# microsoft/hivedscheduler

Hardware: AMD Instinct MI355X
Metric: scheduling p50 latency + VC-safety violations; RCCL bus-bw at 1/2/4/8-GPU cells (lower is better)
Workload: dtype fp32; 1 GPU; model=hived-sched-config4-fragmentation-stress, cluster=simulated 4-node x 8-MI355X, global_batch=64, seq_len=0, parallelism=single

## Files before the change

hivedscheduler_amd/core/algorithm.cpp:

```cpp
#include <cstdio>
#include <cstdlib>

#include "core.hpp"

namespace hived {

bool mapDebugRelease() {
  static int v = -1;
  if (v < 0) v = getenv("HIVED_DEBUG_MAP") ? 1 : 0;
  return v == 1;
}

namespace {
constexpr size_t kWaitReasonReserve = 128;

using OverlappingPreemptors = std::vector<Group*>;

OverlappingPreemptors collectPreemptionVictims(const Placement<PhysicalCell>& placement,
                                               VictimList* victims) {
  OverlappingPreemptors overlapping;
  victims->clear();
  for (auto& [leafNum, pods] : placement) {
    (void)leafNum;
    for (auto& pod : pods) {
// ... 79 lines not shown

int getAllocatedPodIndex(const BindInfo& info, int leafCellNum) {
  for (auto& mbi : info.memberBindInfo) {
    if (mbi.empty() || static_cast<int>(mbi[0].leafIndices.size()) != leafCellNum) continue;
    for (size_t podIndex = 0; podIndex < mbi.size(); podIndex++) {
      auto& pl = mbi[podIndex];
      if (pl.node == info.node && !info.isolation.empty() &&
          std::find(pl.leafIndices.begin(), pl.leafIndices.end(), info.isolation[0]) !=
              pl.leafIndices.end()) {
        return static_cast<int>(podIndex);
      }
    }
  }
  return -1;
}

bool allPodsReleased(const FlatLeafMap<PodSlots>& allocatedPods) {
  for (auto& [ln, pods] : allocatedPods) {
    (void)ln;
    for (auto& p : pods) {
      if (p.present) return false;
    }
  }
  return true;
}

bool anyBoundUnder(PhysicalCell* c) {
  if (c->virt != nullptr) return true;
  for (Cell* ch : c->children) {
    if (anyBoundUnder(static_cast<PhysicalCell*>(ch))) return true;
  }
  return false;
}

void initGroup(Group* g, const PodSpec& s, GState state) {
  g->name = s.groupName;
  g->vc = s.vc;
  g->lazyPreemptionEnable = s.lazyPreemptionEnable;
  g->ignoreK8sSuggestedNodes = s.ignoreK8sSuggestedNodes;
  g->gangReleaseEnable = s.gangReleaseEnable;
  g->priority = s.priority;
  g->state = state;
  g->totalPodNums = s.groupPodNums;
  for (auto& [leafNum, podNum] : s.groupPodNums) {
    g->allocatedPods[leafNum].resize(podNum);
    g->physPlacement[leafNum].assign(podNum, leafNum);
    g->virtPlacement[leafNum].assign(podNum, leafNum);
  }
}

}


ScheduleResult HivedCore::schedule(const PodSpec& s, const std::string& podKey,
                                   const std::set<std::string>& suggestedNodes, Phase phase) {
  OpGuard opGuard(this);
  scheduleCount_++;
  Placement<PhysicalCell> phys;
  Placement<VirtualCell> virt;
  bool hasVirtual = true;
  VictimList& victims = victimScratch_;
  victims.clear();
  std::string waitReason;
  waitReason.reserve(kWaitReasonReserve);
  int podIndex = 0;
  bool havePlacement = false;

  Group* g = nullptr;
  if (auto it = groups_.find(s.groupName); it != groups_.end()) g = it->second.get();
  if (g != nullptr) {
    havePlacement = schedulePodFromExistingGroup(g, s, suggestedNodes, phase, podKey, &phys,
                                                 &hasVirtual, &virt, &victims, &podIndex);
    if (!havePlacement) {
      auto it = groups_.find(s.groupName);
      g = it == groups_.end() ? nullptr : it->second.get();
    }
  }
  if (g == nullptr) {
    g = schedulePodFromNewGroup(s, suggestedNodes, phase, podKey, &phys, &hasVirtual, &virt,
                                &victims, &waitReason);
    havePlacement = !phys.empty();
  }
  (void)havePlacement;
  return generateResult(phys, hasVirtual, virt, victims, std::move(waitReason), s.leafCellNumber,
                        podIndex, g, s.groupName);
}

ScheduleResult HivedCore::generateResult(const Placement<PhysicalCell>& phys, bool hasVirtual,
                                         const Placement<VirtualCell>& virt,
                                         const VictimList& victims,
                                         std::string&& waitReason, int currentLeafNum,
                                         int podIndex, Group* group,
                                         const std::string& groupName) {
  ScheduleResult r;
  if (phys.empty()) {
    r.kind = ScheduleResult::Kind::Wait;
    if (waitReason.empty()) {
      r.waitReason = "waiting for resources";
    } else {
      r.waitReason = std::move(waitReason);
    }
    return r;
  }
  if (!victims.empty()) {
    r.kind = ScheduleResult::Kind::Preempt;
    victims.nodeAt(victimRng_() % victims.nodeCount(), &r.victimNode, &r.victimPodKeys);
    return r;
  }
  r.kind = ScheduleResult::Kind::Bind;
  auto built = std::make_shared<BindInfo>();
  BindInfo& info = *built;
  info.memberBindInfo.reserve(phys.size());
  for (auto& [leafNum, pods] : phys) {
    std::vector<PodPlacementInfo> placements(pods.size());
    for (size_t pi = 0; pi < pods.size(); pi++) {
      auto& pl = placements[pi];
      pl.leafIndices.assign(leafNum, 0);
      pl.preassignedTypes.assign(leafNum, "");
      for (int li = 0; li < leafNum; li++) {
        PhysicalCell* c = pods[pi][li];
        if (c == nullptr) {
          if (group == nullptr || group->state == GState::Preempting) {
// ... 336 lines not shown
      .append(" node");
  return false;
}

bool HivedCore::chainHasBadLinks(const ChainCellList& ccl) {
  for (Cell* c : ccl.at(ccl.top())) {
    if (static_cast<PhysicalCell*>(c)->badLinksUnder > 0) return true;
  }
  return false;
}

std::map<std::string, Placement<VirtualCell>> HivedCore::tryLazyPreempt(
    const Placement<VirtualCell>& p, const std::string& groupName) {
  std::map<std::string, Placement<VirtualCell>> preempted;
  for (auto& [leafNum, pods] : p) {
    (void)leafNum;
    for (auto& pod : pods) {
      for (VirtualCell* leaf : pod) {
        if (PhysicalCell* pc = leaf->phys) {
          if (pc->state == CState::Used && pc->usingGroup->lazyPreemptionEnable &&
              !preempted.count(pc->usingGroup->name)) {
            preempted[pc->usingGroup->name] = lazyPreemptGroup(pc->usingGroup, groupName);
          }
        }
      }
    }
  }
  return preempted;
}

bool HivedCore::scheduleOpportunisticGroup(const SchedulingRequest& sr,
                                           Placement<PhysicalCell>* phys,
                                           std::string* failedReason) {
  if (!sr.topo->Schedule(sr.podLeafCellNums, kOpportunisticPriority, *sr.suggestedNodes,
                         sr.ignoreSuggestedNodes, phys, failedReason, sr.hbmBytes)) {
    failedReason->append(" when scheduling in physical cluster");
    return false;
  }
  return true;
}


void HivedCore::deleteUnallocatedPod(const PodSpec& s, const std::string& podKey) {
  OpGuard opGuard(this);
  auto it = groups_.find(s.groupName);
  if (it == groups_.end() || it->second->state != GState::Preempting) return;
  Group* g = it->second.get();
  g->preemptingPods.erase(podKey);
  if (g->preemptingPods.empty()) {
    deletePreemptingGroup(g, podKey);
  }
}

void HivedCore::addAllocatedPod(const PodSpec& s, const BindInfo& info, const std::string& podKey) {
  addAllocatedPodShared(s, info, nullptr, podKey);
}

void HivedCore::addAllocatedPod(const PodSpec& s, const std::shared_ptr<const BindInfo>& info,
                                const std::string& podKey) {
  addAllocatedPodShared(s, *info, &info, podKey);
}

void HivedCore::addAllocatedPodShared(const PodSpec& s, const BindInfo& info,
                                      const std::shared_ptr<const BindInfo>* shared,
                                      const std::string& podKey) {
  OpGuard opGuard(this);
  int podIndex = 0;
  bool releasable = true;
  Group* g = nullptr;
  auto it = groups_.find(s.groupName);
  if (it != groups_.end()) {
    g = it->second.get();
    if (g->state == GState::Preempting) allocatePreemptingGroup(g, podKey);
    podIndex = getAllocatedPodIndex(info, s.leafCellNumber);
    if (podIndex == -1) return;
  } else {
    g = createAllocatedGroup(s, info, podKey);
    podIndex = getAllocatedPodIndex(info, s.leafCellNumber);
    if (podIndex == -1) {
      podIndex = 0;
      releasable = false;
    }
  }
  setPodSlot(g, s.leafCellNumber, podIndex, releasable, podKey,
             shared != nullptr ? *shared : std::make_shared<const BindInfo>(info));
}

void HivedCore::deleteAllocatedPod(const PodSpec& s, const BindInfo& info,
                                   const std::string& podKey) {
  OpGuard opGuard(this);
  auto it = groups_.find(s.groupName);
  if (it == groups_.end()) return;
  Group* g = it->second.get();
  int podIndex = getAllocatedPodIndex(info, s.leafCellNumber);
  if (podIndex == -1) return;
  clearPodSlot(g, s.leafCellNumber, podIndex);
  if (allPodsReleased(g->allocatedPods)) {
    deleteAllocatedGroup(g, podKey);
  }
}

bool HivedCore::deleteAllocatedPodByKey(const std::string& podKey) {
  auto it = podIndex_.find(podKey);
  if (it == podIndex_.end()) return false;
  const PodSlotRef ref = it->second;
  OpGuard opGuard(this);
  if (!ref.releasable) return true;
  podIndex_.erase(it);
  ref.group->allocatedPods[ref.leafCellNum][ref.podIndex] = AllocatedPod{};
  if (allPodsReleased(ref.group->allocatedPods)) {
    deleteAllocatedGroup(ref.group, podKey);
  }
  return true;
}

void HivedCore::setPodSlot(Group* g, int leafCellNum, int podIndex, bool releasable,
                           const std::string& podKey, std::shared_ptr<const BindInfo> info) {
  auto& slots = g->allocatedPods[leafCellNum];
  if (podIndex >= static_cast<int>(slots.size())) slots.resize(podIndex + 1);
  AllocatedPod& slot = slots[podIndex];
  if (slot.present && slot.key != podKey) clearPodSlot(g, leafCellNum, podIndex);
  slot.present = true;
  slot.key = podKey;
  slot.node = info->node;
  slot.bindInfo = std::move(info);
  podIndex_[podKey] = PodSlotRef{g, leafCellNum, podIndex, releasable};
}

void HivedCore::clearPodSlot(Group* g, int leafCellNum, int podIndex) {
  auto& slots = g->allocatedPods[leafCellNum];
  if (podIndex >= static_cast<int>(slots.size())) return;
  AllocatedPod& slot = slots[podIndex];
  if (slot.present) {
    auto it = podIndex_.find(slot.key);
    if (it != podIndex_.end() && it->second.group == g &&
        it->second.leafCellNum == leafCellNum && it->second.podIndex == podIndex) {
      podIndex_.erase(it);
    }
// ... 442 lines not shown
```

hivedscheduler_amd/core/bindings.cpp:

```cpp
#include <pybind11/pybind11.h>
#include <pybind11/stl.h>

#include <climits>
#include <cstring>
#include <functional>
#include <mutex>

#include "core.hpp"

namespace py = pybind11;
using namespace hived;

namespace {

std::string dstr(const py::dict& d, const char* key, const std::string& def = "") {
  if (!d.contains(key)) return def;
  py::object v = d[key];
  if (v.is_none()) return def;
  return py::cast<std::string>(py::str(v));
}
long long dint(const py::dict& d, const char* key, long long def = 0) {
  if (!d.contains(key)) return def;
  py::object v = d[key];
  if (v.is_none()) return def;
// ... 115 lines not shown
};
Names N{};

PyObject* internName(const char* s) {
  PyObject* o = PyUnicode_InternFromString(s);
  if (o == nullptr) throw py::error_already_set();
  return o;
}

void initNames() {
#define HIVED_NAME(x) N.x = internName(#x)
  HIVED_NAME(virtualCluster);
  HIVED_NAME(priority);
  HIVED_NAME(pinnedCellId);
  HIVED_NAME(leafCellType);
  HIVED_NAME(leafCellNumber);
  HIVED_NAME(gangReleaseEnable);
  HIVED_NAME(lazyPreemptionEnable);
  HIVED_NAME(ignoreK8sSuggestedNodes);
  HIVED_NAME(hbmBytesPerCell);
  HIVED_NAME(affinityGroup);
  HIVED_NAME(name);
  HIVED_NAME(members);
  HIVED_NAME(podNumber);
  HIVED_NAME(node);
  HIVED_NAME(cellChain);
  HIVED_NAME(leafCellIsolation);
  HIVED_NAME(affinityGroupBindInfo);
  HIVED_NAME(podPlacements);
  HIVED_NAME(physicalNode);
  HIVED_NAME(physicalLeafCellIndices);
  HIVED_NAME(preassignedCellTypes);
  HIVED_NAME(kind);
  HIVED_NAME(bind);
  HIVED_NAME(preempt);
  HIVED_NAME(wait);
  HIVED_NAME(bindInfo);
  HIVED_NAME(victimNode);
  HIVED_NAME(victimPodKeys);
  HIVED_NAME(reason);
  HIVED_NAME(pod_spec);
  HIVED_NAME(spec);
  HIVED_NAME(pod_key);
  HIVED_NAME(suggested_nodes);
  HIVED_NAME(phase);
  HIVED_NAME(commit);
  HIVED_NAME(validate);
  HIVED_NAME(Filtering);
  HIVED_NAME(Preempting);
  HIVED_NAME(code);
#undef HIVED_NAME
}

struct ApiTypes {
  PyObject* PodSchedulingSpec;
  PyObject* AffinityGroupSpec;
  PyObject* AffinityGroupMemberSpec;
  PyObject* PodBindInfo;
  PyObject* AffinityGroupMemberBindInfo;
  PyObject* PodPlacementInfo;
  PyObject* WebServerError;
  PyObject* emptyTuple;
  PyObject* one;
};
ApiTypes T{};

void initApiTypes() {
  py::module_ types = py::module_::import("hivedscheduler_amd.api.types");
#define HIVED_TYPE(x) T.x = py::object(types.attr(#x)).release().ptr()
  HIVED_TYPE(PodSchedulingSpec);
  HIVED_TYPE(AffinityGroupSpec);
  HIVED_TYPE(AffinityGroupMemberSpec);
  HIVED_TYPE(PodBindInfo);
  HIVED_TYPE(AffinityGroupMemberBindInfo);
  HIVED_TYPE(PodPlacementInfo);
  HIVED_TYPE(WebServerError);
#undef HIVED_TYPE
  T.emptyTuple = PyTuple_New(0);
  T.one = PyLong_FromLong(1);
  if (T.emptyTuple == nullptr || T.one == nullptr) throw py::error_already_set();
}

class Record {
 public:
  explicit Record(py::handle rec) : rec_(rec.ptr()) {
    if (PyDict_Check(rec_)) {
      dict_ = rec_;
      wire_ = true;
      return;
    }
    PyObject* tp = reinterpret_cast<PyObject*>(Py_TYPE(rec_));
    if (tp == T.PodSchedulingSpec || tp == T.AffinityGroupMemberSpec ||
        tp == T.AffinityGroupSpec) {
      dict_ = ownedDict_ = PyObject_GenericGetDict(rec_, nullptr);
      if (dict_ == nullptr) PyErr_Clear();
    }
  }
  Record(const Record&) = delete;
  Record& operator=(const Record&) = delete;
  ~Record() { Py_XDECREF(ownedDict_); }
  py::handle object() const { return rec_; }

 private:
  friend class Field;
  PyObject* rec_;
  PyObject* dict_ = nullptr;
// ... 252 lines not shown
};

py::dict bindInfoToDict(const BindInfo& info, const NameStrs& names) {
  py::dict d;
  setItem(d, N.node, names.str(info.node));
  setItem(d, N.leafCellIsolation, pyIntList(info.isolation));
  setItem(d, N.cellChain, names.str(info.chain));
  py::list mbis(info.memberBindInfo.size());
  for (size_t m = 0; m < info.memberBindInfo.size(); m++) {
    auto& mbi = info.memberBindInfo[m];
    py::list placements(mbi.size());
    for (size_t p = 0; p < mbi.size(); p++) {
      auto& pl = mbi[p];
      py::dict pd;
      setItem(pd, N.physicalNode, names.str(pl.node));
      setItem(pd, N.physicalLeafCellIndices, pyIntList(pl.leafIndices));
      setItem(pd, N.preassignedCellTypes, names.strList(pl.preassignedTypes));
      PyList_SET_ITEM(placements.ptr(), static_cast<Py_ssize_t>(p), pd.release().ptr());
    }
    py::dict md;
    setItem(md, N.podPlacements, placements);
    PyList_SET_ITEM(mbis.ptr(), static_cast<Py_ssize_t>(m), md.release().ptr());
  }
  setItem(d, N.affinityGroupBindInfo, mbis);
  return d;
}

bool isNodeNameCollection(py::handle v) {
  PyObject* o = v.ptr();
  if (PySequence_Check(o) != 0) return !PyUnicode_Check(o) && !PyBytes_Check(o);
  if (PyGen_Check(o) != 0 || PyAnySet_Check(o) != 0) return true;
  if (PyType_Check(o)) return false;
  const char* tp = Py_TYPE(o)->tp_name;
  for (const char* ok : {"dict_keys", "dict_values", "dict_items", "map", "zip"}) {
    if (std::strcmp(tp, ok) == 0) return true;
  }
  return false;
}

std::set<std::string> toNodeNameSet(py::handle v) {
  std::set<std::string> out;
  Items items(v);
  for (Py_ssize_t i = 0; i < items.size(); i++) {
    py::handle item = items[i];
    if (!PyUnicode_Check(item.ptr()) && !PyBytes_Check(item.ptr())) {
      throw py::type_error("suggested_nodes must contain node names (str)");
    }
    out.insert(py::cast<std::string>(item));
  }
  return out;
}


py::object newInstance(PyObject* cls) {
  PyTypeObject* tp = reinterpret_cast<PyTypeObject*>(cls);
  PyObject* o = tp->tp_new(tp, T.emptyTuple, nullptr);
  if (o == nullptr) throw py::error_already_set();
  return py::reinterpret_steal<py::object>(o);
}
void setAttr(py::handle o, PyObject* name, py::handle value) {
  if (PyObject_SetAttr(o.ptr(), name, value.ptr()) != 0) throw py::error_already_set();
}

py::object defaultAffinityGroup(py::handle podKey, py::handle leafCellNumber) {
  py::object member = newInstance(T.AffinityGroupMemberSpec);
  setAttr(member, N.podNumber, T.one);
  setAttr(member, N.leafCellNumber, leafCellNumber);
  py::list members(1);
  PyList_SET_ITEM(members.ptr(), 0, member.release().ptr());
  py::object group = newInstance(T.AffinityGroupSpec);
  setAttr(group, N.name, podKey);
  setAttr(group, N.members, members);
  return group;
}

PodSpec parseValidatedPodSpec(py::handle spec, py::handle podKey, const std::string& key) {
  if (PyDict_Check(spec.ptr())) {
    throw py::type_error("schedule_pod validates a PodSchedulingSpec object, not a dict");
  }
  Record d(spec);
  PodSpec s;
  Field leaf(d, N.leafCellNumber);
  bool defaulted = false;
  {
    Field ag(d, N.affinityGroup);
    if (!ag) {
      setAttr(spec, N.affinityGroup, defaultAffinityGroup(podKey, leaf.get()));
      defaulted = true;
    }
  }
  s.vc = fstr(d, N.virtualCluster);
  if (s.vc.empty()) throw HivedError::BadRequest("VirtualCluster is empty");
  long long priority = fint(d, N.priority);
  if (priority < kOpportunisticPriority) {
    throw HivedError::BadRequest("Priority is less than " + std::to_string(kOpportunisticPriority));
  }
  if (priority > kMaxGuaranteedPriority) {
    throw HivedError::BadRequest("Priority is greater than " +
                                 std::to_string(kMaxGuaranteedPriority));
  }
  s.priority = static_cast<int>(priority);
  long long leafNum = leaf ? toLongLong(leaf.get()) : 0;
  if (leafNum <= 0) throw HivedError::BadRequest("LeafCellNumber is non-positive");
  s.leafCellNumber = static_cast<int>(leafNum);
  if (defaulted) {
    s.groupName = key;
    s.groupPodNums[s.leafCellNumber] = 1;
  } else {
    Field ag(d, N.affinityGroup);
    Record group(ag.get());
    s.groupName = fstr(group, N.name);
    if (s.groupName.empty()) throw HivedError::BadRequest("AffinityGroup.Name is empty");
    bool podInGroup = false;
    if (Field members{group, N.members}) {
      Items ms(members.get());
      for (Py_ssize_t i = 0; i < ms.size(); i++) {
        Record member(ms[i]);
        long long podNumber = fint(member, N.podNumber);
        if (podNumber <= 0) {
          throw HivedError::BadRequest("AffinityGroup.Members has non-positive PodNumber");
        }
        long long memberLeafNum = fint(member, N.leafCellNumber);
        if (memberLeafNum <= 0) {
          throw HivedError::BadRequest("AffinityGroup.Members has non-positive LeafCellNumber");
        }
        if (memberLeafNum == leafNum) podInGroup = true;
        s.groupPodNums[static_cast<int>(memberLeafNum)] += static_cast<int>(podNumber);
      }
    }
    if (!podInGroup) {
      throw HivedError::BadRequest("AffinityGroup.Members does not contain current Pod");
    }
  }
  s.pinnedCellId = fstr(d, N.pinnedCellId);
  s.leafCellType = fstr(d, N.leafCellType);
  s.gangReleaseEnable = fbool(d, N.gangReleaseEnable, false);
  s.lazyPreemptionEnable = fbool(d, N.lazyPreemptionEnable, false);
  s.ignoreK8sSuggestedNodes = fbool(d, N.ignoreK8sSuggestedNodes, true);
  s.hbmBytesPerCell = fint(d, N.hbmBytesPerCell);
  if (s.hbmBytesPerCell < 0) {
    throw HivedError::BadRequest("hbmBytesPerCell must be non-negative");
  }
  return s;
}

py::object bindInfoToObject(const BindInfo& info, const NameStrs& names) {
  py::list mbis(info.memberBindInfo.size());
  for (size_t m = 0; m < info.memberBindInfo.size(); m++) {
    auto& mbi = info.memberBindInfo[m];
    py::list placements(mbi.size());
    for (size_t p = 0; p < mbi.size(); p++) {
      auto& pl = mbi[p];
      py::object po = newInstance(T.PodPlacementInfo);
      setAttr(po, N.physicalNode, names.str(pl.node));
      setAttr(po, N.physicalLeafCellIndices, pyIntList(pl.leafIndices));
      setAttr(po, N.preassignedCellTypes, names.strList(pl.preassignedTypes));
      PyList_SET_ITEM(placements.ptr(), static_cast<Py_ssize_t>(p), po.release().ptr());
    }
    py::object mo = newInstance(T.AffinityGroupMemberBindInfo);
    setAttr(mo, N.podPlacements, placements);
    PyList_SET_ITEM(mbis.ptr(), static_cast<Py_ssize_t>(m), mo.release().ptr());
  }
  py::object o = newInstance(T.PodBindInfo);
  setAttr(o, N.node, names.str(info.node));
  setAttr(o, N.leafCellIsolation, pyIntList(info.isolation));
  setAttr(o, N.cellChain, names.str(info.chain));
  setAttr(o, N.affinityGroupBindInfo, mbis);
  return o;
}

struct PyScheduleResult {
  PyObject_HEAD
  PyObject* bindInfo;
  PyObject* victimNode;
  PyObject* victimPodKeys;
  PyObject* waitReason;
  hived::ScheduleResult r;
  std::shared_ptr<const NameStrs> names;
};

void resultDealloc(PyObject* self) {
  auto* o = reinterpret_cast<PyScheduleResult*>(self);
  Py_XDECREF(o->bindInfo);
  Py_XDECREF(o->victimNode);
  Py_XDECREF(o->victimPodKeys);
  Py_XDECREF(o->waitReason);
  o->r.~ScheduleResult();
  o->names.~shared_ptr();
  Py_TYPE(self)->tp_free(self);
}

template <class Make>
PyObject* cachedAttr(PyObject** slot, Make make) {
  if (*slot == nullptr) {
    try {
      *slot = make().release().ptr();
    } catch (py::error_already_set& e) {
      e.restore();
      return nullptr;
    } catch (const std::exception& e) {
      PyErr_SetString(PyExc_RuntimeError, e.what());
      return nullptr;
    }
  }
  Py_INCREF(*slot);
  return *slot;
}

PyObject* resultKind(PyObject* self, void*) {
  PyObject* k = nullptr;
  switch (reinterpret_cast<PyScheduleResult*>(self)->r.kind) {
    case hived::ScheduleResult::Kind::Bind: k = N.bind; break;
    case hived::ScheduleResult::Kind::Preempt: k = N.preempt; break;
    case hived::ScheduleResult::Kind::Wait: k = N.wait; break;
  }
  Py_INCREF(k);
  return k;
}
PyObject* resultBindInfo(PyObject* self, void*) {
  auto* o = reinterpret_cast<PyScheduleResult*>(self);
  if (o->r.kind != hived::ScheduleResult::Kind::Bind) Py_RETURN_NONE;
// ... 253 lines not shown
    if (!isNodeNameCollection(suggestedNodes)) {
      throw py::type_error("suggested_nodes must be a sequence of node names, not " +
                           std::string(Py_TYPE(suggestedNodes.ptr())->tp_name));
    }
    PodSpec s = parsePodSpec(spec);
    bool needSuggested = !s.ignoreK8sSuggestedNodes;
    if (!needSuggested) {
      CoreSection section(coreMutex_);
      auto it = core_.groups().find(s.groupName);
      needSuggested = it != core_.groups().end() && !it->second->ignoreK8sSuggestedNodes;
    }
    std::set<std::string> suggested;
    if (needSuggested) suggested = toNodeNameSet(suggestedNodes);
    Phase ph = (phase == "Preempting") ? Phase::Preempting : Phase::Filtering;
    ScheduleResult r = [&] {
      CoreSection section(coreMutex_);
      return core_.schedule(s, podKey, suggested, ph);
    }();
    py::dict d;
    switch (r.kind) {
      case ScheduleResult::Kind::Bind:
        setItem(d, N.kind, N.bind);
        setItem(d, N.bindInfo, bindInfoToDict(*r.bindInfo, *nameStrs_));
        break;
      case ScheduleResult::Kind::Preempt:
        setItem(d, N.kind, N.preempt);
        setItem(d, N.victimNode, pyStr(r.victimNode));
        setItem(d, N.victimPodKeys, pyStrList(r.victimPodKeys));
        break;
      case ScheduleResult::Kind::Wait:
        setItem(d, N.kind, N.wait);
        setItem(d, N.reason, pyStr(r.waitReason));
        break;
    }
    return d;
  }

  py::object schedulePod(py::handle spec, py::handle podKey, py::handle suggestedNodes,
                         py::handle phase, bool commit, bool validate) {
    if (!PyUnicode_Check(podKey.ptr())) throw py::type_error("pod_key must be a str");
    Phase ph = Phase::Filtering;
    if (phase.ptr() != nullptr && phase.ptr() != N.Filtering) {
      if (!PyUnicode_Check(phase.ptr())) throw py::type_error("phase must be a str");
      if (phase.ptr() == N.Preempting ||
          PyUnicode_CompareWithASCIIString(phase.ptr(), "Preempting") == 0) {
        ph = Phase::Preempting;
      }
    }
    if (!suggestedNodes.is_none() && !isNodeNameCollection(suggestedNodes)) {
      throw py::type_error("suggested_nodes must be a sequence of node names, not " +
                           std::string(Py_TYPE(suggestedNodes.ptr())->tp_name));
    }
    std::string key = toStdString(podKey);
    PodSpec s = validate ? parseValidatedPodSpec(spec, podKey, key) : parsePodSpec(spec);
    bool needSuggested = !s.ignoreK8sSuggestedNodes;
    if (!needSuggested) {
      CoreSection section(coreMutex_);
      auto it = core_.groups().find(s.groupName);
      needSuggested = it != core_.groups().end() && !it->second->ignoreK8sSuggestedNodes;
    }
    std::set<std::string> given;
    const std::set<std::string>* suggested = &given;
    if (needSuggested) {
      if (suggestedNodes.is_none()) {
        suggested = &allNodeSet_;
      } else {
        given = toNodeNameSet(suggestedNodes);
      }
    }
    hived::ScheduleResult r = [&] {
      CoreSection section(coreMutex_);
      hived::ScheduleResult decided = core_.schedule(s, key, *suggested, ph);
      if (commit && decided.kind == hived::ScheduleResult::Kind::Bind) {
        core_.addAllocatedPod(s, decided.bindInfo, key);
      }
      return decided;
    }();
    return makeResult(std::move(r), nameStrs_);
  }

  void deleteUnallocatedPod(py::handle spec, const std::string& podKey) {
    PodSpec s = parsePodSpec(spec);
    CoreSection section(coreMutex_);
    core_.deleteUnallocatedPod(s, podKey);
  }
  void addAllocatedPod(py::handle spec, py::handle bindInfo, const std::string& podKey) {
    PodSpec s = parsePodSpec(spec);
    BindInfo info = parseBindInfo(bindInfo);
    CoreSection section(coreMutex_);
    core_.addAllocatedPod(s, info, podKey);
  }
  void deleteAllocatedPod(py::handle spec, py::handle bindInfo, const std::string& podKey) {
    PodSpec s = parsePodSpec(spec);
    BindInfo info = parseBindInfo(bindInfo);
    CoreSection section(coreMutex_);
    core_.deleteAllocatedPod(s, info, podKey);
  }

  bool deleteAllocatedPodByKey(py::handle podKey) {
    if (!PyUnicode_Check(podKey.ptr())) throw py::type_error("pod_key must be a str");
    Py_ssize_t n = 0;
    const char* utf8 = PyUnicode_AsUTF8AndSize(podKey.ptr(), &n);
    if (utf8 == nullptr) throw py::error_already_set();
    CoreSection section(coreMutex_);
    releaseKey_.assign(utf8, static_cast<size_t>(n));
    return core_.deleteAllocatedPodByKey(releaseKey_);
  }

  py::list getAllAffinityGroups() const {
    py::list out;
    for (auto& [name, g] : core_.groups()) {
      (void)name;
      out.append(groupToDict(g.get()));
    }
    return out;
  }

  py::dict getAffinityGroup(const std::string& name) const {
    auto it = core_.groups().find(name);
    if (it == core_.groups().end()) {
      throw HivedError::BadRequest("Affinity group " + name +
                                   " does not exist since it is not allocated or preempting");
    }
    return groupToDict(it->second.get());
  }

  py::dict getClusterStatus() {
    py::dict d;
    d["physicalCluster"] = getPhysicalClusterStatus();
    d["virtualClusters"] = getAllVirtualClustersStatus();
    return d;
// ... 45 lines not shown
      (void)chain;
      for (Cell* c : st.full.at(kLowestLevel)) {
        auto* pc = static_cast<PhysicalCell*>(c);
        if (pc->otVC == vcName) {
          py::dict d;
          d["cellType"] = pc->typeName;
          d["cellAddress"] = pc->address + "-opp";
          d["cellState"] = to_string(CState::Used);
          d["cellHealthiness"] = pc->healthy ? "Healthy" : "Bad";
          d["cellPriority"] = kOpportunisticPriority;
          d["physicalCell"] = pc->address;
          out.append(d);
        }
      }
    }
    return out;
  }

  long long scheduleCount() const { return core_.scheduleCount_; }
  void checkInvariants() const { hived::checkInvariants(core_); }

  py::dict debugCounters() const {
    py::dict d;
    for (auto& [chain, st] : core_.chainStates_) {
      py::dict cd;
      for (int level = kLowestLevel; level <= st.top; level++) {
        py::dict ld;
        ld["totalLeft"] = st.totalLeft[level];
        ld["allVCFree"] = st.allVCFree[level];
        py::dict vd;
        for (const VCChainState* vcc : st.vcs) {
          if (vcc->free[level] != 0) vd[py::str(vcc->vc)] = vcc->free[level];
        }
        ld["vcFree"] = vd;
        py::list fl;
        for (auto* fc : st.free.at(level)) fl.append(fc->address);
        ld["freeList"] = fl;
        if (st.allVCDoomedBadCellNum[level] != 0) ld["doomed"] = st.allVCDoomedBadCellNum[level];
        ld["badFree"] = static_cast<int>(st.badFree.at(level).size());
        cd[py::int_(level)] = ld;
      }
      d[py::str(chain)] = cd;
    }
    return d;
  }

 private:
  HivedCore core_;
  std::vector<py::object> nodeNames_;
  std::shared_ptr<const NameStrs> nameStrs_;
  std::set<std::string> allNodeSet_;
  CoreMutex coreMutex_;
  std::string releaseKey_;
};


PyObject* gCoreError = nullptr;
PyTypeObject* gCoreType = nullptr;

PyObject* newCoreError(const HivedError& e) {
  PyObject* text = PyUnicode_FromString(e.what());
  if (text == nullptr) return nullptr;
  PyObject* inst = PyObject_CallFunctionObjArgs(gCoreError, text, nullptr);
  Py_DECREF(text);
  if (inst == nullptr) return nullptr;
  PyObject* code = PyLong_FromLong(e.code);
  if (code == nullptr || PyObject_SetAttr(inst, N.code, code) != 0) {
    Py_XDECREF(code);
    Py_DECREF(inst);
    return nullptr;
  }
  Py_DECREF(code);
  return inst;
}

void setCoreError(const HivedError& e, bool asWebServerError) {
  PyObject* inst = newCoreError(e);
  if (inst == nullptr) return;
  if (!asWebServerError) {
    PyErr_SetObject(gCoreError, inst);
    Py_DECREF(inst);
    return;
  }
  PyObject* web = PyObject_CallFunction(T.WebServerError, "is", e.code, e.what());
  if (web == nullptr) {
    Py_DECREF(inst);
    return;
  }
  Py_INCREF(inst);
  PyException_SetCause(web, inst);
  PyException_SetContext(web, inst);
  PyErr_SetObject(T.WebServerError, web);
  Py_DECREF(web);
}

bool toFlag(PyObject* o, const char* name) {
  if (o == Py_True) return true;
  if (o == Py_False || o == Py_None) return false;
  PyNumberMethods* num = Py_TYPE(o)->tp_as_number;
  if (num != nullptr && num->nb_bool != nullptr) {
    int r = num->nb_bool(o);
    if (r < 0) throw py::error_already_set();
    return r != 0;
  }
  throw py::type_error(std::string(name) + " must be a bool");
}
// ... 127 lines not shown
                           PyObject* kwnames) {
  return deleteByKeyCall(self, args, nargs, kwnames, false);
}
PyObject* deleteValidatedByKeyEntry(PyObject* self, PyObject* const* args, Py_ssize_t nargs,
                                    PyObject* kwnames) {
  return deleteByKeyCall(self, args, nargs, kwnames, true);
}

using FastCallWithKeywords = PyObject* (*)(PyObject*, PyObject* const*, Py_ssize_t, PyObject*);
PyCFunction asCFunction(FastCallWithKeywords f) {
  return reinterpret_cast<PyCFunction>(reinterpret_cast<void (*)()>(f));
}

PyMethodDef directMethods[] = {
    {"schedule_pod", asCFunction(schedulePodEntry), METH_FASTCALL | METH_KEYWORDS,
     "schedule_pod($self, /, pod_spec, pod_key, suggested_nodes=None, phase='Filtering', "
     "commit=False, validate=True)\n--\n\n"
     "One filter decision in one call: validate and default the request, decide,\n"
     "commit a bind decision, return the native ScheduleResult. Raises CoreError."},
    {"schedule_validated_pod", asCFunction(scheduleValidatedPodEntry),
     METH_FASTCALL | METH_KEYWORDS,
     "schedule_validated_pod($self, /, spec, pod_key, suggested_nodes=None, "
     "phase='Filtering', commit=False)\n--\n\n"
     "schedule_pod with validate=True whose core errors leave as\n"
     "WebServerError(code, text) with the CoreError as __cause__."},
    {"delete_allocated_pod_by_key", asCFunction(deleteByKeyEntry), METH_FASTCALL | METH_KEYWORDS,
     "delete_allocated_pod_by_key($self, /, pod_key)\n--\n\n"
     "Release the allocated pod the core holds under pod_key, as\n"
     "delete_allocated_pod does for the spec and bind info it was added with.\n"
     "False, and nothing changed, if the core holds no such pod. Raises CoreError."},
    {"delete_validated_pod_by_key", asCFunction(deleteValidatedByKeyEntry),
     METH_FASTCALL | METH_KEYWORDS,
     "delete_validated_pod_by_key($self, /, pod_key)\n--\n\n"
     "delete_allocated_pod_by_key whose core errors leave as\n"
     "WebServerError(code, text) with the CoreError as __cause__."},
};

void addDirectMethods(py::handle cls) {
  gCoreType = reinterpret_cast<PyTypeObject*>(cls.ptr());
  for (PyMethodDef& def : directMethods) {
    PyObject* descr = PyDescr_NewMethod(gCoreType, &def);
    if (descr == nullptr) throw py::error_already_set();
    int rc = PyObject_SetAttrString(cls.ptr(), def.ml_name, descr);
    Py_DECREF(descr);
    if (rc != 0) throw py::error_already_set();
  }
}

}

PYBIND11_MODULE(hivedcore, m) {
  m.doc() = "MI355X-native gang scheduler core (C++)";
  initNames();
  initApiTypes();
  initResultType(m);

  static py::exception<HivedError> exc(m, "CoreError");
  gCoreError = exc.ptr();
  py::register_exception_translator([](std::exception_ptr p) {
    try {
      if (p) std::rethrow_exception(p);
    } catch (const HivedError& e) {
      py::object pyExc = exc;
      py::object inst = pyExc(e.what());
      inst.attr("code") = e.code;
      PyErr_SetObject(pyExc.ptr(), inst.ptr());
    }
  });

  py::class_<PyHivedCore> coreClass(m, "HivedCore");
  coreClass
      .def(py::init<const py::dict&>(), py::arg("spec"))
      .def("set_node_healthy", &PyHivedCore::setNodeHealthy, py::arg("node"), py::arg("healthy"))
      .def("set_xgmi_link_healthy", &PyHivedCore::setXgmiLinkHealthy, py::arg("node"),
           py::arg("a"), py::arg("b"), py::arg("healthy"), py::arg("gbps") = 0.0)
      .def("xgmi_links", &PyHivedCore::xgmiLinks, py::arg("node"))
      .def("set_leaf_cell_healthy", &PyHivedCore::setLeafCellHealthy, py::arg("node"),
           py::arg("leaf_index"), py::arg("healthy"))
      .def("all_nodes", &PyHivedCore::allNodes)
      .def("bad_nodes", &PyHivedCore::badNodes)
      .def("schedule", &PyHivedCore::schedule, py::arg("pod_spec"), py::arg("pod_key"),
           py::arg("suggested_nodes"), py::arg("phase"))
      .def("delete_unallocated_pod", &PyHivedCore::deleteUnallocatedPod, py::arg("pod_spec"),
           py::arg("pod_key"))
      .def("add_allocated_pod", &PyHivedCore::addAllocatedPod, py::arg("pod_spec"),
           py::arg("bind_info"), py::arg("pod_key"))
      .def("delete_allocated_pod", &PyHivedCore::deleteAllocatedPod, py::arg("pod_spec"),
           py::arg("bind_info"), py::arg("pod_key"))
      .def("get_all_affinity_groups", &PyHivedCore::getAllAffinityGroups)
      .def("get_affinity_group", &PyHivedCore::getAffinityGroup, py::arg("name"))
      .def("get_cluster_status", &PyHivedCore::getClusterStatus)
      .def("get_physical_cluster_status", &PyHivedCore::getPhysicalClusterStatus)
      .def("get_all_virtual_clusters_status", &PyHivedCore::getAllVirtualClustersStatus)
      .def("get_virtual_cluster_status", &PyHivedCore::getVirtualClusterStatus, py::arg("vc"))
      .def("schedule_count", &PyHivedCore::scheduleCount)
      .def("check_invariants", &PyHivedCore::checkInvariants)
      .def("debug_counters", &PyHivedCore::debugCounters);
  addDirectMethods(coreClass);
}
```

hivedscheduler_amd/core/core.hpp:

```cpp
#pragma once

#include <algorithm>
#include <cstddef>
#include <map>
#include <memory>
#include <new>
#include <optional>
#include <random>
#include <set>
#include <stdexcept>
#include <string>
#include <unordered_map>
#include <unordered_set>
#include <vector>

namespace hived {

constexpr int kMaxGuaranteedPriority = 1000;
constexpr int kMinGuaranteedPriority = 0;
constexpr int kOpportunisticPriority = -1;
constexpr int kFreePriority = -2;
constexpr int kLowestLevel = 1;
constexpr int kHighestLevel = 100;

// ... 791 lines not shown
  void seal() {
    auto less = [](const Entry& a, const Entry& b) {
      const int c = a.first->compare(*b.first);
      return c != 0 ? c < 0 : *a.second < *b.second;
    };
    auto same = [](const Entry& a, const Entry& b) {
      return *a.first == *b.first && *a.second == *b.second;
    };
    std::sort(pods_.begin(), pods_.end(), less);
    pods_.erase(std::unique(pods_.begin(), pods_.end(), same), pods_.end());
    nodes_ = 0;
    for (size_t i = 0; i < pods_.size(); i++) {
      if (i == 0 || *pods_[i].first != *pods_[i - 1].first) nodes_++;
    }
  }
  size_t nodeCount() const { return nodes_; }
  void nodeAt(size_t index, std::string* node, std::vector<std::string>* keys) const {
    size_t at = 0;
    size_t i = 0;
    for (; i < pods_.size(); i++) {
      if (i > 0 && *pods_[i].first != *pods_[i - 1].first) at++;
      if (at == index) break;
    }
    *node = *pods_[i].first;
    size_t last = i;
    while (last < pods_.size() && *pods_[last].first == *node) last++;
    keys->clear();
    keys->reserve(last - i);
    for (; i < last; i++) keys->push_back(*pods_[i].second);
  }

 private:
  using Entry = std::pair<const std::string*, const std::string*>;
  std::vector<Entry> pods_;
  size_t nodes_ = 0;
};

using CellBindings = SmallPtrMap<VirtualCell, PhysicalCell*, 32>;

class HivedCore {
 public:
  explicit HivedCore(const ClusterSpec& spec);
  ~HivedCore();

  void setNodeHealthy(const std::string& node, bool healthy);
  void setLeafCellHealthy(const std::string& node, int leafIndex, bool healthy);
  void setXgmiLinkHealthy(const std::string& node, int a, int b, bool healthy,
                          double gbps = 0.0);
  std::vector<std::tuple<int, int, double, bool>> xgmiLinks(const std::string& node) const;
  std::vector<std::string> allNodes() const;
  std::set<std::string> badNodes() const { return badNodes_; }

  ScheduleResult schedule(const PodSpec& s, const std::string& podKey,
                          const std::set<std::string>& suggestedNodes, Phase phase);
  void deleteUnallocatedPod(const PodSpec& s, const std::string& podKey);
  void addAllocatedPod(const PodSpec& s, const BindInfo& info, const std::string& podKey);
  void addAllocatedPod(const PodSpec& s, const std::shared_ptr<const BindInfo>& info,
                       const std::string& podKey);
  void deleteAllocatedPod(const PodSpec& s, const BindInfo& info, const std::string& podKey);
  bool deleteAllocatedPodByKey(const std::string& podKey);

  const std::map<std::string, std::unique_ptr<Group>>& groups() const { return groups_; }
  const std::map<std::string, IntraVCScheduler>& vcSchedulers() const { return vcSchedulers_; }
  std::vector<std::string> chains() const;
  std::map<int, std::string> chainLevelTypes(const std::string& chain) const;

 private:
  friend struct BuildContext;

  void buildFromSpec(const ClusterSpec& spec);
  void initCellNums();
  void initPinnedCells();
  void initBadNodes();

  void setBadCell(PhysicalCell* c);
  void setHealthyCell(PhysicalCell* c);
  void addBadFreeCell(PhysicalCell* c);
  void removeBadFreeCell(PhysicalCell* c);
  bool doomAllocationIsSafe(PhysicalCell* pc);
  void tryBindDoomedBadCell(ChainState* chain, int level);
  void tryUnbindDoomedBadCell(ChainState* chain, int level);
  void doBindDoomedBadCell(ChainState* chain, int level);
  void doUnbindDoomedBadCell(ChainState* chain, int level);
  void drainDoomChecks();

  class OpGuard {
   public:
    explicit OpGuard(HivedCore* c)
        : c_(c), outer_(!c->inOperation_), exceptionsAtEntry_(std::uncaught_exceptions()) {
      c_->inOperation_ = true;
    }
    ~OpGuard() noexcept(false) {
      if (!outer_) return;
      c_->inOperation_ = false;
      if (std::uncaught_exceptions() == exceptionsAtEntry_) c_->drainDoomChecks();
    }

   private:
    HivedCore* c_;
    bool outer_;
    int exceptionsAtEntry_;
  };

  ScheduleResult generateResult(const Placement<PhysicalCell>& phys, bool hasVirtual,
                                const Placement<VirtualCell>& virt,
                                const VictimList& victims,
                                std::string&& waitReason, int currentLeafNum, int podIndex,
                                Group* group, const std::string& groupName);
  bool schedulePodFromExistingGroup(Group* g, const PodSpec& s,
                                    const std::set<std::string>& suggestedNodes, Phase phase,
                                    const std::string& podKey, Placement<PhysicalCell>* phys,
                                    bool* hasVirtual, Placement<VirtualCell>* virt,
                                    VictimList* victims,
                                    int* podIndex);
  Group* schedulePodFromNewGroup(const PodSpec& s, const std::set<std::string>& suggestedNodes,
                                 Phase phase, const std::string& podKey,
                                 Placement<PhysicalCell>* phys, bool* hasVirtual,
                                 Placement<VirtualCell>* virt,
                                 VictimList* victims,
                                 std::string* waitReason);
  bool scheduleNewAffinityGroup(const PodSpec& s, const std::set<std::string>& suggestedNodes,
                                const std::string& podKey, Placement<PhysicalCell>* phys,
                                bool* hasVirtual, Placement<VirtualCell>* virt,
                                std::string* failedReason);
  bool scheduleForLeafCellType(SchedulingRequest& sr, const std::string& leafCellType,
                               const std::vector<ChainState*>& chains,
                               const std::string& podKey, bool typeSpecified,
                               Placement<PhysicalCell>* phys, bool* hasVirtual,
                               Placement<VirtualCell>* virt, std::string* failedReason);
  bool handleSchedulingRequest(SchedulingRequest& sr, Placement<PhysicalCell>* phys,
                               bool* hasVirtual, Placement<VirtualCell>* virt,
                               std::string* failedReason);
  bool scheduleGuaranteedGroup(SchedulingRequest& sr, Placement<PhysicalCell>* phys,
                               Placement<VirtualCell>* virt, std::string* failedReason);
  static bool chainHasBadLinks(const ChainCellList& fullCells);
  bool scheduleOpportunisticGroup(const SchedulingRequest& sr, Placement<PhysicalCell>* phys,
                                  std::string* failedReason);
  void validateSchedulingRequest(SchedulingRequest& sr, const std::string& podKey);

  std::map<std::string, Placement<VirtualCell>> tryLazyPreempt(const Placement<VirtualCell>& p,
                                                               const std::string& groupName);

  void addAllocatedPodShared(const PodSpec& s, const BindInfo& info,
                             const std::shared_ptr<const BindInfo>* shared,
                             const std::string& podKey);
  void setPodSlot(Group* g, int leafCellNum, int podIndex, bool releasable,
                  const std::string& podKey, std::shared_ptr<const BindInfo> info);
  void clearPodSlot(Group* g, int leafCellNum, int podIndex);
  void eraseGroup(Group* g);
  Group* insertNewGroup(const PodSpec& s, GState state);

  Group* createAllocatedGroup(const PodSpec& s, const BindInfo& info, const std::string& podKey);
  void deleteAllocatedGroup(Group* g, const std::string& podKey);
  Group* createPreemptingGroup(const PodSpec& s, const Placement<PhysicalCell>& phys,
                               const Placement<VirtualCell>& virt, const std::string& podKey);
  void deletePreemptingGroup(Group* g, const std::string& podKey);
  void allocatePreemptingGroup(Group* g, const std::string& podKey);
  Placement<VirtualCell> lazyPreemptGroup(Group* victim, const std::string& preemptor);
  void lazyPreemptCell(VirtualCell* c, const std::string& preemptor);
  void revertLazyPreempt(Group* g, const Placement<VirtualCell>& virt);

  std::pair<PhysicalCell*, VirtualCell*> findAllocatedLeafCell(
      int index, const PodPlacementInfo& placement, const std::string& chain, const PodSpec& s,
      const IntraVCScheduler* vcs, const std::vector<PhysicalCell*>* nodeLeaves, Group* group,
      const std::string& podKey, bool* lazyPreempt, bool* isOpportunistic);
  std::pair<bool, std::string> allocateLeafCell(PhysicalCell* p, VirtualCell* v, int priority,
                                                const std::string& vc);
  void releaseLeafCell(PhysicalCell* p, const std::string& vc);
  std::pair<bool, std::string> allocatePreassignedCell(PhysicalCell* c, VCChainState* vc,
                                                       bool doomedBad);
  void releasePreassignedCell(PhysicalCell* c, VCChainState* vc, bool doomedBad);
  void allocateBadCell(PhysicalCell* c);
  void releaseBadCell(PhysicalCell* c);
  int removeCellFromFreeList(PhysicalCell* c);
  int addCellToFreeList(PhysicalCell* c);

  bool mapVirtualPlacementToPhysical(const std::vector<BindingVertex*>& preassigned,
                                     const std::vector<std::vector<BindingVertex*>>& nonPreassigned,
                                     size_t nonPreassignedCount, ChainCellList& freeList,
                                     std::vector<int>& freeCellNum,
                                     const std::set<std::string>& suggestedNodes,
                                     bool ignoreSuggestedNodes, CellBindings& bindings,
                                     long long minHbmBytes = 0, bool honorLinks = false,
                                     const CleanShapeWorld* world = nullptr);

  struct MapScratch {
    std::vector<std::unique_ptr<BindingVertex>> vertexPool;
    size_t verticesUsed = 0;
    std::vector<BindingVertex*> preassigned;
    std::vector<std::vector<BindingVertex*>> nonPreassigned;
    size_t nonPreassignedUsed = 0;
    std::vector<VirtualCell*> path;
    ChainCellList freeList;
    std::vector<int> freeCellNum;
    void reset() {
      verticesUsed = 0;
// ... 77 lines not shown
```

Measured before the change: 711.0 ns.

## Fill Python result objects directly and reuse group lookup across schedule call

Python result objects (bind info, placements, affinity groups) are now built by creating the instance dict directly and inserting fields, instead of issuing one setattr call per field. The schedule path also reuses the group found while checking ignoreK8sSuggestedNodes as a hint, so the core skips a second map lookup and the whole decision runs in one locked section. Boundary counters and a bool return from addAllocatedPod are added for introspection. Writing to the instance dict directly bypasses descriptors or __setattr__ on those classes, and it uses a private CPython API.

```diff
diff --git a/hivedscheduler_amd/core/algorithm.cpp b/hivedscheduler_amd/core/algorithm.cpp
--- a/hivedscheduler_amd/core/algorithm.cpp
+++ b/hivedscheduler_amd/core/algorithm.cpp
@@ -155,8 +155,8 @@
 }
 
 
-ScheduleResult HivedCore::schedule(const PodSpec& s, const std::string& podKey,
-                                   const std::set<std::string>& suggestedNodes, Phase phase) {
+ScheduleResult HivedCore::scheduleFrom(Group* g, const PodSpec& s, const std::string& podKey,
+                                       const std::set<std::string>& suggestedNodes, Phase phase) {
   OpGuard opGuard(this);
   scheduleCount_++;
   Placement<PhysicalCell> phys;
@@ -169,8 +169,6 @@
   int podIndex = 0;
   bool havePlacement = false;
 
-  Group* g = nullptr;
-  if (auto it = groups_.find(s.groupName); it != groups_.end()) g = it->second.get();
   if (g != nullptr) {
     havePlacement = schedulePodFromExistingGroup(g, s, suggestedNodes, phase, podKey, &phys,
                                                  &hasVirtual, &virt, &victims, &podIndex);
@@ -613,16 +611,16 @@
   }
 }
 
-void HivedCore::addAllocatedPod(const PodSpec& s, const BindInfo& info, const std::string& podKey) {
-  addAllocatedPodShared(s, info, nullptr, podKey);
-}
-
-void HivedCore::addAllocatedPod(const PodSpec& s, const std::shared_ptr<const BindInfo>& info,
+bool HivedCore::addAllocatedPod(const PodSpec& s, const BindInfo& info, const std::string& podKey) {
+  return addAllocatedPodShared(s, info, nullptr, podKey);
+}
+
+bool HivedCore::addAllocatedPod(const PodSpec& s, const std::shared_ptr<const BindInfo>& info,
                                 const std::string& podKey) {
-  addAllocatedPodShared(s, *info, &info, podKey);
-}
-
-void HivedCore::addAllocatedPodShared(const PodSpec& s, const BindInfo& info,
+  return addAllocatedPodShared(s, *info, &info, podKey);
+}
+
+bool HivedCore::addAllocatedPodShared(const PodSpec& s, const BindInfo& info,
                                       const std::shared_ptr<const BindInfo>* shared,
                                       const std::string& podKey) {
   OpGuard opGuard(this);
@@ -630,11 +628,12 @@
   bool releasable = true;
   Group* g = nullptr;
   auto it = groups_.find(s.groupName);
-  if (it != groups_.end()) {
+  const bool created = it == groups_.end();
+  if (!created) {
     g = it->second.get();
     if (g->state == GState::Preempting) allocatePreemptingGroup(g, podKey);
     podIndex = getAllocatedPodIndex(info, s.leafCellNumber);
-    if (podIndex == -1) return;
+    if (podIndex == -1) return false;
   } else {
     g = createAllocatedGroup(s, info, podKey);
     podIndex = getAllocatedPodIndex(info, s.leafCellNumber);
@@ -645,6 +644,7 @@
   }
   setPodSlot(g, s.leafCellNumber, podIndex, releasable, podKey,
              shared != nullptr ? *shared : std::make_shared<const BindInfo>(info));
+  return created;
 }
 
 void HivedCore::deleteAllocatedPod(const PodSpec& s, const BindInfo& info,
diff --git a/hivedscheduler_amd/core/bindings.cpp b/hivedscheduler_amd/core/bindings.cpp
--- a/hivedscheduler_amd/core/bindings.cpp
+++ b/hivedscheduler_amd/core/bindings.cpp
@@ -191,6 +191,27 @@
 #undef HIVED_NAME
 }
 
+PyObject* groupFields[2];
+PyObject* memberFields[2];
+PyObject* bindInfoFields[4];
+PyObject* memberBindFields[1];
+PyObject* placementFields[3];
+
+void initFieldLists() {
+  groupFields[0] = N.name;
+  groupFields[1] = N.members;
+  memberFields[0] = N.podNumber;
+  memberFields[1] = N.leafCellNumber;
+  bindInfoFields[0] = N.node;
+  bindInfoFields[1] = N.leafCellIsolation;
+  bindInfoFields[2] = N.cellChain;
+  bindInfoFields[3] = N.affinityGroupBindInfo;
+  memberBindFields[0] = N.podPlacements;
+  placementFields[0] = N.physicalNode;
+  placementFields[1] = N.physicalLeafCellIndices;
+  placementFields[2] = N.preassignedCellTypes;
+}
+
 struct ApiTypes {
   PyObject* PodSchedulingSpec;
   PyObject* AffinityGroupSpec;
@@ -549,34 +570,55 @@
 }
 
 
-py::object newInstance(PyObject* cls) {
-  PyTypeObject* tp = reinterpret_cast<PyTypeObject*>(cls);
-  PyObject* o = tp->tp_new(tp, T.emptyTuple, nullptr);
-  if (o == nullptr) throw py::error_already_set();
-  return py::reinterpret_steal<py::object>(o);
-}
 void setAttr(py::handle o, PyObject* name, py::handle value) {
   if (PyObject_SetAttr(o.ptr(), name, value.ptr()) != 0) throw py::error_already_set();
 }
 
+py::object newInstance(PyObject* cls, PyObject* const* names, PyObject* const* values, int n) {
+  PyTypeObject* tp = reinterpret_cast<PyTypeObject*>(cls);
+  PyObject* raw = tp->tp_new(tp, T.emptyTuple, nullptr);
+  if (raw == nullptr) throw py::error_already_set();
+  py::object o = py::reinterpret_steal<py::object>(raw);
+#ifndef HIVED_NO_DIRECT_FILL
+  PyObject** slot = _PyObject_GetDictPtr(raw);
+  if (slot != nullptr && *slot == nullptr) {
+    PyObject* d = PyDict_New();
+    if (d == nullptr) throw py::error_already_set();
+    *slot = d;
+    for (int i = 0; i < n; i++) {
+      if (PyDict_SetItem(d, names[i], values[i]) != 0) throw py::error_already_set();
+    }
+    return o;
+  }
+#endif
+  for (int i = 0; i < n; i++) setAttr(o, names[i], values[i]);
+  return o;
+}
+
 py::object defaultAffinityGroup(py::handle podKey, py::handle leafCellNumber) {
-  py::object member = newInstance(T.AffinityGroupMemberSpec);
-  setAttr(member, N.podNumber, T.one);
-  setAttr(member, N.leafCellNumber, leafCellNumber);
+  PyObject* const memberValues[2] = {T.one, leafCellNumber.ptr()};
+  py::object member = newInstance(T.AffinityGroupMemberSpec, memberFields, memberValues, 2);
   py::list members(1);
   PyList_SET_ITEM(members.ptr(), 0, member.release().ptr());
-  py::object group = newInstance(T.AffinityGroupSpec);
-  setAttr(group, N.name, podKey);
-  setAttr(group, N.members, members);
-  return group;
-}
-
-PodSpec parseValidatedPodSpec(py::handle spec, py::handle podKey, const std::string& key) {
+  PyObject* const groupValues[2] = {podKey.ptr(), members.ptr()};
+  return newInstance(T.AffinityGroupSpec, groupFields, groupValues, 2);
+}
+
+struct BoundaryCounters {
+  long long fastReads = 0;
+  long long slowReads = 0;
+  long long fastCommits = 0;
+  long long slowCommits = 0;
+};
+
+PodSpec parseValidatedPodSpec(py::handle spec, py::handle podKey, const std::string& key,
+                              BoundaryCounters* counters) {
   if (PyDict_Check(spec.ptr())) {
     throw py::type_error("schedule_pod validates a PodSchedulingSpec object, not a dict");
   }
+  PodSpec s;
+  counters->slowReads++;
   Record d(spec);
-  PodSpec s;
   Field leaf(d, N.leafCellNumber);
   bool defaulted = false;
   {
@@ -648,22 +690,22 @@
     py::list placements(mbi.size());
     for (size_t p = 0; p < mbi.size(); p++) {
       auto& pl = mbi[p];
-      py::object po = newInstance(T.PodPlacementInfo);
-      setAttr(po, N.physicalNode, names.str(pl.node));
-      setAttr(po, N.physicalLeafCellIndices, pyIntList(pl.leafIndices));
-      setAttr(po, N.preassignedCellTypes, names.strList(pl.preassignedTypes));
+      py::object node = names.str(pl.node);
+      py::object indices = pyIntList(pl.leafIndices);
+      py::object types = names.strList(pl.preassignedTypes);
+      PyObject* const values[3] = {node.ptr(), indices.ptr(), types.ptr()};
+      py::object po = newInstance(T.PodPlacementInfo, placementFields, values, 3);
       PyList_SET_ITEM(placements.ptr(), static_cast<Py_ssize_t>(p), po.release().ptr());
     }
-    py::object mo = newInstance(T.AffinityGroupMemberBindInfo);
-    setAttr(mo, N.podPlacements, placements);
+    PyObject* const values[1] = {placements.ptr()};
+    py::object mo = newInstance(T.AffinityGroupMemberBindInfo, memberBindFields, values, 1);
     PyList_SET_ITEM(mbis.ptr(), static_cast<Py_ssize_t>(m), mo.release().ptr());
   }
-  py::object o = newInstance(T.PodBindInfo);
-  setAttr(o, N.node, names.str(info.node));
-  setAttr(o, N.leafCellIsolation, pyIntList(info.isolation));
-  setAttr(o, N.cellChain, names.str(info.chain));
-  setAttr(o, N.affinityGroupBindInfo, mbis);
-  return o;
+  py::object node = names.str(info.node);
+  py::object isolation = pyIntList(info.isolation);
+  py::object chain = names.str(info.chain);
+  PyObject* const values[4] = {node.ptr(), isolation.ptr(), chain.ptr(), mbis.ptr()};
+  return newInstance(T.PodBindInfo, bindInfoFields, values, 4);
 }
 
 struct PyScheduleResult {
@@ -1023,31 +1065,57 @@
                            std::string(Py_TYPE(suggestedNodes.ptr())->tp_name));
     }
     std::string key = toStdString(podKey);
-    PodSpec s = validate ? parseValidatedPodSpec(spec, podKey, key) : parsePodSpec(spec);
-    bool needSuggested = !s.ignoreK8sSuggestedNodes;
-    if (!needSuggested) {
+    PodSpec s = validate ? parseValidatedPodSpec(spec, podKey, key, &boundary_) : parsePodSpec(spec);
+    return makeResult(decideInSections(s, key, suggestedNodes, ph, commit), nameStrs_);
+  }
+
+ private:
+  hived::ScheduleResult decideAndCommit(const PodSpec& s, const std::string& key,
+                                        const std::set<std::string>& suggested, Phase ph,
+                                        bool commit, const HivedCore::GroupHint* found) {
+    hived::ScheduleResult decided = found != nullptr
+                                        ? core_.schedule(s, key, suggested, ph, *found)
+                                        : core_.schedule(s, key, suggested, ph);
+    if (commit && decided.kind == hived::ScheduleResult::Kind::Bind) {
+      if (core_.addAllocatedPod(s, decided.bindInfo, key)) boundary_.slowCommits++;
+    }
+    return decided;
+  }
+
+  hived::ScheduleResult decideInSections(const PodSpec& s, const std::string& key,
+                                         py::handle suggestedNodes, Phase ph, bool commit) {
+    std::set<std::string> given;
+    if (s.ignoreK8sSuggestedNodes) {
       CoreSection section(coreMutex_);
       auto it = core_.groups().find(s.groupName);
-      needSuggested = it != core_.groups().end() && !it->second->ignoreK8sSuggestedNodes;
-    }
-    std::set<std::string> given;
+      Group* found = it == core_.groups().end() ? nullptr : it->second.get();
+      if (found == nullptr || found->ignoreK8sSuggestedNodes) {
+#ifndef HIVED_NO_GROUP_HINT
+        const HivedCore::GroupHint hint{found};
+        return decideAndCommit(s, key, given, ph, commit, &hint);
+#else
+        return decideAndCommit(s, key, given, ph, commit, nullptr);
+#endif
+      }
+    }
     const std::set<std::string>* suggested = &given;
-    if (needSuggested) {
-      if (suggestedNodes.is_none()) {
-        suggested = &allNodeSet_;
-      } else {
-        given = toNodeNameSet(suggestedNodes);
-      }
-    }
-    hived::ScheduleResult r = [&] {
-      CoreSection section(coreMutex_);
-      hived::ScheduleResult decided = core_.schedule(s, key, *suggested, ph);
-      if (commit && decided.kind == hived::ScheduleResult::Kind::Bind) {
-        core_.addAllocatedPod(s, decided.bindInfo, key);
-      }
-      return decided;
-    }();
-    return makeResult(std::move(r), nameStrs_);
+    if (suggestedNodes.is_none()) {
+      suggested = &allNodeSet_;
+    } else {
+      given = toNodeNameSet(suggestedNodes);
+    }
+    CoreSection section(coreMutex_);
+    return decideAndCommit(s, key, *suggested, ph, commit, nullptr);
+  }
+
+ public:
+  py::dict boundaryCounters() const {
+    py::dict d;
+    d["fast_reads"] = boundary_.fastReads;
+    d["slow_reads"] = boundary_.slowReads;
+    d["fast_commits"] = boundary_.fastCommits;
+    d["slow_commits"] = boundary_.slowCommits;
+    return d;
   }
 
   void deleteUnallocatedPod(py::handle spec, const std::string& podKey) {
@@ -1199,6 +1267,7 @@
   std::set<std::string> allNodeSet_;
   CoreMutex coreMutex_;
   std::string releaseKey_;
+  BoundaryCounters boundary_;
 };
 
 
@@ -1432,6 +1501,7 @@
 PYBIND11_MODULE(hivedcore, m) {
   m.doc() = "MI355X-native gang scheduler core (C++)";
   initNames();
+  initFieldLists();
   initApiTypes();
   initResultType(m);
 
@@ -1475,6 +1545,7 @@
       .def("get_virtual_cluster_status", &PyHivedCore::getVirtualClusterStatus, py::arg("vc"))
       .def("schedule_count", &PyHivedCore::scheduleCount)
       .def("check_invariants", &PyHivedCore::checkInvariants)
-      .def("debug_counters", &PyHivedCore::debugCounters);
+      .def("debug_counters", &PyHivedCore::debugCounters)
+      .def("boundary_counters", &PyHivedCore::boundaryCounters);
   addDirectMethods(coreClass);
 }
diff --git a/hivedscheduler_amd/core/core.hpp b/hivedscheduler_amd/core/core.hpp
--- a/hivedscheduler_amd/core/core.hpp
+++ b/hivedscheduler_amd/core/core.hpp
@@ -867,10 +867,22 @@
   std::set<std::string> badNodes() const { return badNodes_; }
 
   ScheduleResult schedule(const PodSpec& s, const std::string& podKey,
-                          const std::set<std::string>& suggestedNodes, Phase phase);
+                          const std::set<std::string>& suggestedNodes, Phase phase) {
+    auto it = groups_.find(s.groupName);
+    return scheduleFrom(it == groups_.end() ? nullptr : it->second.get(), s, podKey,
+                        suggestedNodes, phase);
+  }
+  struct GroupHint {
+    Group* group;
+  };
+  ScheduleResult schedule(const PodSpec& s, const std::string& podKey,
+                          const std::set<std::string>& suggestedNodes, Phase phase,
+                          GroupHint found) {
+    return scheduleFrom(found.group, s, podKey, suggestedNodes, phase);
+  }
   void deleteUnallocatedPod(const PodSpec& s, const std::string& podKey);
-  void addAllocatedPod(const PodSpec& s, const BindInfo& info, const std::string& podKey);
-  void addAllocatedPod(const PodSpec& s, const std::shared_ptr<const BindInfo>& info,
+  bool addAllocatedPod(const PodSpec& s, const BindInfo& info, const std::string& podKey);
+  bool addAllocatedPod(const PodSpec& s, const std::shared_ptr<const BindInfo>& info,
                        const std::string& podKey);
   void deleteAllocatedPod(const PodSpec& s, const BindInfo& info, const std::string& podKey);
   bool deleteAllocatedPodByKey(const std::string& podKey);
@@ -917,6 +929,8 @@
     int exceptionsAtEntry_;
   };
 
+  ScheduleResult scheduleFrom(Group* g, const PodSpec& s, const std::string& podKey,
+                              const std::set<std::string>& suggestedNodes, Phase phase);
   ScheduleResult generateResult(const Placement<PhysicalCell>& phys, bool hasVirtual,
                                 const Placement<VirtualCell>& virt,
                                 const VictimList& victims,
@@ -956,7 +970,7 @@
   std::map<std::string, Placement<VirtualCell>> tryLazyPreempt(const Placement<VirtualCell>& p,
                                                                const std::string& groupName);
 
-  void addAllocatedPodShared(const PodSpec& s, const BindInfo& info,
+  bool addAllocatedPodShared(const PodSpec& s, const BindInfo& info,
                              const std::shared_ptr<const BindInfo>* shared,
                              const std::string& podKey);
   void setPodSlot(Group* g, int leafCellNum, int podIndex, bool releasable,
```

Result: no change. 711.0 ns (+0.0%).
